# cityflow-project/CityFlow

Measured on AMD Instinct MI355X. Metric: vehicle_steps_per_sec, higher is better.
Workload: dtype f64; 1 GPU; grid_30x30 (reference generator, --tlPlan, interval 1.0) + 3000 seeded interior flows (1 veh / 6 s each until t=240 s); single engine; running_vehicles_start=96748, running_vehicles_end=71131, lanes=11160, lane_count_hash_end=cf8592fdc74305bd, backend=hip-gfx950, layout=ring, parallelism=1 gpu

## Files before the change

cityflow_amd/csrc/hip/cfx_kernels.h:

```cpp
#pragma once

#include "cfx_device.h"

namespace cfxd {

constexpr int kBlock = 256;
#ifndef CFX_ACT_BLOCK
#define CFX_ACT_BLOCK 64
#endif
#ifndef CFX_CROSS_BLOCK
#define CFX_CROSS_BLOCK 256
#endif
constexpr int kActBlock = CFX_ACT_BLOCK;
constexpr int kCrossBlock = CFX_CROSS_BLOCK;
#ifndef CFX_LDS_TEMPL
#define CFX_LDS_TEMPL 32
#endif
constexpr int kLdsTempl = CFX_LDS_TEMPL;
template <class T> __device__ __forceinline__ T ldsRead(const T *p) { return *(const __attribute__((address_space(3))) T *) p; }
template <bool GT>
__device__ __forceinline__ const cfx_vehicle_template *templatesOf(const DevTables &t, cfx_vehicle_template *sT) {
    if constexpr (GT) {
        return t.templ;
    } else {
        const int nd = t.nTempl * (int) (sizeof(cfx_vehicle_template) / sizeof(double));
        const double *src = (const double *) t.templ;
        double *dst = (double *) sT;
        for (int i = threadIdx.x; i < nd; i += blockDim.x) dst[i] = src[i];
        return sT;
    }
}
#ifndef CFX_SCATTER_WAVES
#define CFX_SCATTER_WAVES 0
#endif
#ifndef CFX_SCAN_WAVES
#define CFX_SCAN_WAVES 0
#endif
#if CFX_SCAN_WAVES > 0
#define CFX_SCAN_BOUNDS __launch_bounds__(kBlock, CFX_SCAN_WAVES)
#else
#define CFX_SCAN_BOUNDS __launch_bounds__(kBlock)
#endif
#if CFX_SCATTER_WAVES > 0
#define CFX_SCATTER_BOUNDS __launch_bounds__(kBlock, CFX_SCATTER_WAVES)
#else
#define CFX_SCATTER_BOUNDS
#endif

struct VidTable {
    int32_t *priority, *templ, *route, *nextWait;
    double *enterTime;
    double *customSpeed;
    double *gapState;
    uint8_t *state;
    uint8_t *pendingCustom;
    int32_t *firstNext;
};
constexpr int kFirstNextUnknown = -3;
template <class C>
__device__ __forceinline__ void admittedNext(const C &c, int fn, int lane, int road, int laneIdx, int route, int *next, int *onLast) {
    if (fn != kFirstNextUnknown) {
        *next = fn >= 0 ? fn : -1;
        *onLast = fn == -2 ? 2 : 0;
        return;
    }
    const int base = c.t.routeStart[route];
    if (c.t.routeRoads[base] == road) {
        const int ll = c.t.nextLL[c.t.nextStart[base] + laneIdx];
        *next = ll < 0 ? -1 : c.n.L + ll;
    } else {
        *next = nextOf(c.n, c.t, lane, route, 0);
    }
    *onLast = (*next < 0 && isLastRoad(c, lane, route)) ? 2 : 0;
}

struct DevScalars {
    long long active;
    long long finishedCnt;
    double cumulativeTravelTime;
    long long vehicleSteps;
    int nFinishedStep;
    int overflow;
    int nCrossJobs;
    int nLeftUncounted;
    int ringNearFull;
    int actionMaxT;
    long long tieEvents;
    int tieDrv[8];
    long long admitPending[2];
    int crossJobsStep;
    int crossMultiPass;
    int crossMaxPasses;
    int actionMultiPass;
};

struct HostMirror {
    DevScalars sc;
    int32_t slots;
    int32_t pad;
    unsigned long long progress;
};

struct CompactScratch {
    int32_t *leaveCnt;
    int32_t *maxLeaveIdx;
    int32_t *inCnt;
    int32_t *inHead;
    int32_t *inNext;
};

constexpr int kJobShards = 16;
constexpr int kJobShardStride = 32;
constexpr int kFinShards = 16;
struct FinMap {
    int end[kFinShards];
};
__device__ inline int finMapLoad(FinMap &m, const int32_t *finCount, int finCap) {
    if (threadIdx.x == 0) {
        const int capShard = finCap / kFinShards;
        int run = 0;
        for (int i = 0; i < kFinShards; ++i) {
            run += min(finCount[i * 32], capShard);
            m.end[i] = run;
        }
    }
    __syncthreads();
    return m.end[kFinShards - 1];
}
__device__ __forceinline__ int finAt(const FinMap &m, int finCap, int i) {
    int sh = 0;
    while (i >= m.end[sh]) ++sh;
    return sh * (finCap / kFinShards) + (i - (sh ? m.end[sh - 1] : 0));
}
__device__ __forceinline__ void finCountsClear(int32_t *finCount) {
    for (int i = 0; i < kFinShards; ++i) finCount[i * 32] = 0;
}
__device__ __forceinline__ int finPlace(int32_t *finCount, int finCap) {
    const int shard = blockIdx.x & (kFinShards - 1), capShard = finCap / kFinShards;
    const int idx = atomicAdd(&finCount[shard * 32], 1);
    return idx < capShard ? shard * capShard + idx : -1;
}

struct JobQueue {
    int32_t *count;
    int32_t *jobs;
    int capacity;
    int32_t *overflow;
};

struct ActionBuf {
    double *dis, *speed;
    int32_t *drv;
    int32_t *blocker;
};

__global__ void k_spawn_link(const cfx_spawn *recs, int n, int firstNewVid, VidTable vt, int32_t *waitHead, LcDev lc) {
    int i = blockIdx.x * blockDim.x + threadIdx.x;
    if (i >= n) return;
    cfx_spawn r = recs[i];
    if (lc.on) lcInitVid(lc, r.vid);
    vt.priority[r.vid] = r.priority;
    vt.templ[r.vid] = r.templ;
    vt.route[r.vid] = r.route;
    vt.enterTime[r.vid] = r.enter_time;
    vt.state[r.vid] = 0;
    vt.pendingCustom[r.vid] = 0;
    vt.firstNext[r.vid] = kFirstNextUnknown;
    if (r.lane < 0) return;
    if (r.prev_wait < 0) {
        waitHead[r.lane] = r.vid;
    } else if (r.prev_wait >= firstNewVid) {
        vt.nextWait[r.prev_wait] = r.vid;
    } else if (vt.state[r.prev_wait] != 0) {
        waitHead[r.lane] = r.vid;
    } else {
        vt.nextWait[r.prev_wait] = r.vid;
    }
}

__device__ __forceinline__ int lcNaiveSegment(const StepCtx &c, int lane, double dis) {
    const int nSeg = c.lc.laneNumSegs[lane];
// ... 3082 lines not shown
```

cityflow_amd/csrc/hip/cfx_ring_kernels.h:

```cpp
#pragma once

#include <type_traits>

#include "cfx_kernels.h"


namespace cfxd {

struct RingCtx {
#ifndef CFX_RING_CROSS2_WAVES
#define CFX_RING_CROSS2_WAVES 5
#endif
    static constexpr int kCross2Waves = CFX_RING_CROSS2_WAVES;
    DevNet n;
    DevTables t;
    SlotArrays s;
    double2 *kin;
    double2 *kinN;
    int4 *meta;
    const int2 *blkR;
    int2 *blkW;
    int32_t *slotOf;
    const uint8_t *vState;
    const int2 *ringGeo;
// ... 88 lines not shown
}
__device__ __forceinline__ double2 ntLoad2(const double2 *p) {
    const cfx_v2d v = __builtin_nontemporal_load((const cfx_v2d *) p);
    return make_double2(v.x, v.y);
}
__device__ __forceinline__ void ntStore4(int4 *p, int4 x) {
    const cfx_v4i v = {x.x, x.y, x.z, x.w};
    __builtin_nontemporal_store(v, (cfx_v4i *) p);
}
__device__ __forceinline__ void ntStore2(double2 *p, double a, double b) {
    const cfx_v2d v = {a, b};
    __builtin_nontemporal_store(v, (cfx_v2d *) p);
}

struct RingOut {
    double2 *kinN;
    int2 *blk;
    int4 *scratch;
    MoverRec *movers;
    DevScalars *sc;
    long long *finKey;
    int32_t *finVid;
    int finCap;
    int32_t *finCount;
    __device__ __forceinline__ void park(int s, double v, double iv) const { kinN[s] = make_double2(iv, v); }
    __device__ __forceinline__ double parkedSpeed(int s) const { return kinN[s].y; }
    __device__ __forceinline__ double parkedInterSpeed(int s) const { return kinN[s].x; }
    __device__ __forceinline__ void keep(int s, double dis, double speed) const { kinN[s] = make_double2(dis, speed); }
};
constexpr int kRingIdxBits = 20;

template <bool LC>
__device__ inline void finishAction(const RingCtx &c, const RingOut &o, const cfx_vehicle_template &t, int s, int d, int ,
                                    double speed, double dis, double dlen, int nd0, double v, int blockerSlot, int idx = -1,
                                    int nNow = -1, LeaverPrefetch lp = LeaverPrefetch{false, 0.0, 0, 0, 0}, int flags = -1) {
    static_assert(!LC, "the ring layout does not run lane change");
    v = min2(v, 100);
    if (nd0 < 0) {
        const bool lastRoad = flags >= 0 ? (flags & 2) != 0 : isLastRoad(c, d, c.s.route[s]);
        if (!lastRoad) v = min2(v, noCollisionSpeed(0, 1, speed, t.max_neg_acc, dlen - dis, c.interval, t.min_gap));
    }
    v = max2(v, speed - t.max_neg_acc * c.interval);
    double deltaDis;
    if (v < 0) {
        deltaDis = 0.5 * speed * speed / t.max_neg_acc;
        v = 0;
    } else {
        deltaDis = (speed + v) * c.interval / 2;
    }
    double ndis = deltaDis + dis;
    int newDrv = -1;
    if (ndis > dlen) {
        if (!lp.valid) {
            lp.nextLen = nd0 >= 0 ? c.n.drvLength[nd0] : 0.0;
            lp.vid = c.s.vid[s];
            lp.route = c.s.route[s];
            lp.routePos = c.s.routePos[s];
        }
        ndis -= dlen;
        int drivable = nd0;
        newDrv = drivable >= 0 ? drivable : -2;
        if (drivable >= 0 && ndis > lp.nextLen) {
            int nxt = nextOf(c.n, c.t, drivable, lp.route, lp.routePos);
            for (;;) {
                ndis -= c.n.drvLength[drivable];
                drivable = nxt;
                newDrv = drivable >= 0 ? drivable : -2;
                if (drivable < 0 || !(ndis > c.n.drvLength[drivable])) break;
                nxt = nextOf(c.n, c.t, drivable, lp.route, lp.routePos);
            }
        }
    }
    const int bv = blockerSlot >= 0 ? (lp.blockerVidP2 > 0 ? lp.blockerVidP2 - 2 : c.s.vid[blockerSlot]) : -1;
    if (idx < 0) {
        const int2 geo = c.ringGeo[d];
        idx = (s - geo.x - c.head[d]) & geo.y;
        nNow = cntNow(c, d);
    }
    if (newDrv == -1) {
        if (CFX_KL_NT & 4) ntStore2(&o.kinN[s], ndis, v);
        else o.kinN[s] = make_double2(ndis, v);
        if (bv >= 0) o.blk[s] = make_int2(bv, c.step);
        if (idx == nNow - 1) {
            TailRec r;
            r.dis = ndis;
            r.speed = v;
            r.slot = s;
            r.templ = lp.templP1 > 0 ? lp.templP1 - 1 : c.meta[s].x;
            r.prevDrv = lp.prevValid ? lp.prevDrv : c.s.prevDrv[s];
            r.tag = c.step;
            c.tailW[d] = r;
        }
        return;
    }
    o.kinN[s].y = -1.0;
    atomicAdd(&o.scratch[d].x, 1);
    atomicMax(&o.scratch[d].y, idx);
    if (newDrv >= 0) {
        MoverRec r;
        r.vid = lp.vid;
        r.templ = lp.templP1 > 0 ? lp.templP1 - 1 : c.meta[s].x;
        r.route = lp.route;
        r.routePos = lp.routePos;
        r.oldDrv = d;
        r.newDrv = newDrv;
        r.blockerVid = bv;
        r.dis = ndis;
        r.speed = v;
        atomicAdd(&o.scratch[newDrv].w, 1);
        r.nextIn = atomicExch(&o.scratch[newDrv].z, s);
        o.movers[s] = r;
    } else {
        const int f = finPlace(o.finCount, o.finCap);
        if (f >= 0) {
            o.finKey[f] = ((long long) d << kRingIdxBits) | idx;
            o.finVid[f] = lp.vid;
        } else {
            o.sc->overflow = 1;
        }
    }
}

static_assert(sizeof(SpawnBatch) + sizeof(RingCtx) + sizeof(VidTable) + 256 <= 8192, "kr_admit's arguments: a few KB (the runtime takes 32 KB and more, tools/kernarg_probe.hip)");

struct RingCommit {
    int4 *scratch;
    const MoverRec *movers;
    int32_t *waitHead;
    int32_t *curPhase;
    double *remain;
    int rlTrafficLight, nMaskWords;
    DevScalars *sc;
    const long long *finKey;
    const int32_t *finVid;
    double *finTerm;
    int finCap;
    int32_t *jobCount;
    HostMirror *hostMirror;
    int32_t *finTicket;
    int nStatBlocks;
    uint8_t *vStateW;
    int32_t *slotOfW;
    int exactTimes;
    int lightsDone;
    int32_t *hostCnt;
    int32_t *finCount;
};
struct CommitOut {
    int touched, head, n, tailWritten;
    int entrants;
    TailRec tail;
};
__device__ inline void commitDrivable(const RingCtx &c, const RingCommit &k, const int d, CommitOut *out = nullptr);
__device__ inline void commitStatBlock(const RingCtx &c, const RingCommit &k, const VidTable &vt, int part);
__device__ inline int commitStatBlocks(const RingCommit &k);
__device__ inline void commitClearMasks(const RingCtx &c, const RingCommit &k, int gid, int stride);

struct RingHalo {
    int on;
    const int32_t *cutIndex;
    HaloDev h;
    HaloIO io;
    long long *activeOut;
};

__device__ inline int ringHaloGlobalPrev(const RingCtx &c, const HaloDev &h, int prevDrv) {
    if (prevDrv >= c.n.L) return h.llGlobal[prevDrv - c.n.L];
    if (prevDrv <= -2) return -prevDrv - 2;
    return -1;
}

__device__ inline void ringHaloExport(const RingCtx &c, const RingCommit &k, const RingHalo &rh, int d, int ci, const CommitOut &co) {
    const HaloDev &h = rh.h;
    const int2 geo = c.ringGeo[d];
    int head = co.touched ? co.head : c.head[d];
    int n = co.touched ? co.n : c.cnt[d];
    if (ci < h.nGhost) {
        char *blk = rh.io.send[h.ghostPeer[ci]] + h.ghostSendOff[ci];
        const int in = co.entrants;
        int m = in;
        if (m > CFX_HALO_MAX_MIGRANTS) {
            m = CFX_HALO_MAX_MIGRANTS;
            k.sc->overflow = 3;
        }
        ((int32_t *) blk)[0] = m;
        ((int32_t *) blk)[1] = 0;
        HaloMigrant *rec = (HaloMigrant *) (blk + 8);
        for (int j = 0; j < m; ++j) {
            const int s = ringSlot(geo, head, n - in + j);
            const double2 kv = c.kinN[s];
            HaloMigrant r;
            r.vid = c.s.vid[s];
            r.routePos = c.s.routePos[s];
            r.prevLL = ringHaloGlobalPrev(c, h, c.s.prevDrv[s]);
            r.pad = 0;
            r.dis = kv.x;
            r.speed = kv.y;
            rec[j] = r;
        }
        h.ghostHadEntrants[ci] = in > 0;
        if (in > 0) {
            for (int j = 0; j + 1 < n; ++j) c.slotOf[c.s.vid[ringSlot(geo, head, j)]] = -1;
            head = (head + n - 1) & geo.y;
            c.head[d] = head;
            c.cnt[d] = 1;
            atomicAdd((unsigned long long *) rh.activeOut, (unsigned long long) in);
        }
        return;
    }
    const int j = ci - h.nGhost;
    if (j < h.nImport) {
        HaloTail t;
        t.vid = -1;
        t.prevLL = -1;
        t.dis = 0.0;
        t.speed = 0.0;
        if (n > 0) {
            const int s = ringSlot(geo, head, n - 1);
            const double2 kv = c.kinN[s];
            t.vid = c.s.vid[s];
            t.prevLL = ringHaloGlobalPrev(c, h, c.s.prevDrv[s]);
            t.dis = kv.x;
            t.speed = kv.y;
        }
        *(HaloTail *) (rh.io.send[h.importPeer[j]] + h.importSendOff[j]) = t;
    }
}

__device__ inline void ringHaloWriteTail(const RingCtx &c, int lane, int slot) {
    TailRec r{};
    r.slot = -1;
    if (slot >= 0) {
        const double2 kv = c.kin[slot];
        r.dis = kv.x;
        r.speed = kv.y;
        r.slot = slot;
        r.templ = c.meta[slot].x;
        r.prevDrv = c.s.prevDrv[slot];
    }
    r.tag = c.step - 1;
    const_cast<TailRec *>(c.tailR)[lane] = r;
}

__device__ inline void ringHaloImportCut(const RingCtx &c, const HaloDev &h, const HaloIO &io, const VidTable &vt, DevScalars *sc, int i) {
    if (i < h.nImport) {
        const int l = h.importLane[i];
        const char *blk = io.recv[h.importPeer[i]] + h.importRecvOff[i];
        const int m = ((const int32_t *) blk)[0];
        if (m <= 0) return;
        const HaloMigrant *rec = (const HaloMigrant *) (blk + 8);
        const int2 geo = c.ringGeo[l];
        const int head = c.head[l], n = c.cnt[l];
        if (n + m > geo.y) {
            sc->overflow = 8;
            return;
        }
        const int road = c.n.laneRoad[l];
        int last = -1;
        for (int j = 0; j < m; ++j) {
            const HaloMigrant r = rec[j];
            const int s = ringSlot(geo, head, n + j);
            const int route = vt.route[r.vid];
            const int next = nextOf(c.n, c.t, l, route, r.routePos);
            const int base = c.t.routeStart[route], len = c.t.routeStart[route + 1] - base;
            const int onLast = (next < 0 && c.t.routeRoads[base + len - 1] == road) ? 2 : 0;
            c.s.vid[s] = r.vid;
            c.s.drv[s] = l;
            c.s.prevDrv[s] = r.prevLL >= 0 ? -(r.prevLL + 2) : -1;
            c.s.routePos[s] = r.routePos;
            c.s.route[s] = route;
            c.meta[s] = make_int4(vt.templ[r.vid], next, onLast, CFX_INT_MAX);
            c.kin[s] = make_double2(r.dis, r.speed);
            const_cast<int2 *>(c.blkR)[s] = make_int2(-1, -1);
            c.slotOf[r.vid] = s;
            vt.state[r.vid] = 1;
            last = s;
        }
        c.cnt[l] = n + m;
        atomicAdd((unsigned long long *) &sc->active, (unsigned long long) m);
        ringHaloWriteTail(c, l, last);
        return;
    }
    const int j = i - h.nImport;
    if (j < h.nGhost && !h.ghostHadEntrants[j]) {
        const int g = h.ghostLane[j];
        const HaloTail t = *(const HaloTail *) (io.recv[h.ghostPeer[j]] + h.ghostRecvOff[j]);
        const int2 geo = c.ringGeo[g];
        const int head = c.head[g], n = c.cnt[g];
        for (int q = 0; q < n; ++q) {
            const int v = c.s.vid[ringSlot(geo, head, q)];
            if (v != t.vid) c.slotOf[v] = -1;
        }
        if (t.vid < 0) {
            c.cnt[g] = 0;
            ringHaloWriteTail(c, g, -1);
            return;
        }
        int prev = -1;
        if (t.prevLL >= 0) {
            const int k = h.llLocalOfGlobal[t.prevLL];
            prev = k >= 0 ? c.n.L + k : -(t.prevLL + 2);
        }
        const int s = ringSlot(geo, head, 0);
        c.s.vid[s] = t.vid;
        c.s.drv[s] = g;
        c.s.prevDrv[s] = prev;
        c.s.routePos[s] = 0;
        c.s.route[s] = vt.route[t.vid];
        c.meta[s] = make_int4(vt.templ[t.vid], -1, 0, CFX_INT_MAX);
        c.kin[s] = make_double2(t.dis, t.speed);
        const_cast<int2 *>(c.blkR)[s] = make_int2(-1, -1);
        c.slotOf[t.vid] = s;
        c.cnt[g] = 1;
        ringHaloWriteTail(c, g, s);
    }
}

__device__ inline bool ringHaloWaitPeer(const HaloIO &io, int p, DevScalars *sc) {
    unsigned spins = 0;
    while (__hip_atomic_load(io.waitFlag[p], __ATOMIC_ACQUIRE, __HIP_MEMORY_SCOPE_SYSTEM) < io.epoch) {
        if (++spins > (1u << 22)) {
            sc->overflow = 4;
            return false;
        }
        __builtin_amdgcn_s_sleep(16);
    }
    return true;
}

struct RingHaloIn {
    int on;
    const int32_t *cutIndex;
    HaloDev h;
    HaloIO io;
    long long *activeOut;
};

__global__ void kr_halo_import(RingCtx c, HaloDev h, HaloIO io, VidTable vt, DevScalars *sc, long long *activeOut) {
    if (io.nWait > 0) {
        __shared__ int ok;
        if (threadIdx.x == 0) {
            ok = 1;
            for (int p = 0; p < io.nWait && ok; ++p) ok = ringHaloWaitPeer(io, p, sc) ? 1 : 0;
        }
        __syncthreads();
        if (!ok) return;
    }
    const int i = blockIdx.x * blockDim.x + threadIdx.x;
    if (i == 0) {
        const long long out = *activeOut;
        if (out) {
            *activeOut = 0;
            atomicAdd((unsigned long long *) &sc->active, (unsigned long long) (-out));
        }
    }
    if (i < h.nImport + h.nGhost) ringHaloImportCut(c, h, io, vt, sc, i);
}

template <bool COMMIT, int NB = kAdmitRecs, class Batch = SpawnBatchT<NB>, bool GT = false>
__global__ __launch_bounds__(kBlock) void kr_admit(RingCtx cIn, int32_t *admitStep, int32_t *waitHead, VidTable vt, DevScalars *sc,
                                                   const Batch batch, const RingCommit k, const RingHaloIn hin) {
    constexpr bool kMem = std::is_same<Batch, SpawnBatchMem>::value;
    const int d = blockIdx.x * blockDim.x + threadIdx.x;
    const bool isLane = d < cIn.n.L, inRange = d < cIn.n.L + cIn.n.K;
    int b0 = 0, b1 = 0;
    if constexpr (kMem) {
        if ((int) blockIdx.x < batch.nLaneBlocks) {
            b0 = batch.blockOff[blockIdx.x];
            b1 = batch.blockOff[blockIdx.x + 1];
        }
    }
    TailRec committed{};
    int w = -1, n = 0, head = 0, road = 0, laneIdx = 0;
    int2 geo = make_int2(0, 0);
    int wt = 0, route = 0, nextWait = -1, fn = kFirstNextUnknown;
    uint8_t pending = 0;
    if constexpr (COMMIT) {
        const int nBody = (int) gridDim.x - commitStatBlocks(k);
        if ((int) blockIdx.x >= nBody) {
            commitStatBlock(cIn, k, vt, (int) blockIdx.x - nBody);
            return;
        }
        commitClearMasks(cIn, k, d, nBody * (int) blockDim.x);
        if (inRange) committed = cIn.tailW[d];
        if (isLane) {
            w = waitHead[d];
            if (admitStep[d] == cIn.step) w = cIn.admitRec[d].y;
            n = cIn.cnt[d];
            geo = cIn.ringGeo[d];
            head = cIn.head[d];
            road = cIn.n.laneRoad[d];
            laneIdx = cIn.n.laneIndex[d];
            if (w >= 0) {
                wt = vt.templ[w];
                route = vt.route[w];
                nextWait = vt.nextWait[w];
                pending = vt.pendingCustom[w];
                fn = vt.firstNext[w];
            }
        }
        if (inRange) {
            CommitOut co;
            commitDrivable(cIn, k, d, &co);
            if (co.touched) {
                head = co.head;
                n = co.n;
                if (co.tailWritten) committed = co.tail;
            }
        }
    }
    RingCtx c = cIn;
    if constexpr (!COMMIT) {
        if (hin.on) {
            if (d == 0) {
                const long long out = *hin.activeOut;
                if (out) {
                    *hin.activeOut = 0;
                    atomicAdd((unsigned long long *) &sc->active, (unsigned long long) (-out));
                }
            }
            const int ci = isLane ? hin.cutIndex[d] : -1;
            if (ci >= 0) {
                const int nG = hin.h.nGhost;
                const int peer = ci < nG ? hin.h.ghostPeer[ci] : hin.h.importPeer[ci - nG];
                if (hin.io.nWait == 0 || ringHaloWaitPeer(hin.io, peer, sc))
                    ringHaloImportCut(c, hin.h, hin.io, vt, sc, ci < nG ? hin.h.nImport + ci : ci - nG);
            }
        }
    }
    if constexpr (COMMIT) {
        c.step = cIn.step + 1;
        c.tailR = cIn.tailW;
        c.tailW = const_cast<TailRec *>(cIn.tailR);
        c.kin = cIn.kinN;
        c.kinN = cIn.kin;
        c.blkR = cIn.blkW;
        c.blkW = const_cast<int2 *>(cIn.blkR);
    }
    __shared__ int sAdmitted;
    __shared__ cfx_vehicle_template sT[kLdsTempl];
    __shared__ int sLane[NB];
    const int nRecs = batch.n, firstNewVid = batch.firstNewVid;
    if (threadIdx.x == 0) sAdmitted = 0;
    if constexpr (kMem) {
        for (int i = threadIdx.x; i < b1 - b0 && i < NB; i += blockDim.x) sLane[i] = batch.lane[b0 + i];
    } else {
        for (int i = threadIdx.x; i < nRecs; i += blockDim.x) sLane[i] = batch.lane[i];
    }
    auto laneOfRec = [&](int j) {
        if constexpr (kMem) return j - b0 < NB ? ldsRead(&sLane[j - b0]) : batch.lane[j];
        else return sLane[j];
    };
    const int recLo = kMem ? b0 : 0, recHi = kMem ? b1 : nRecs;
    const cfx_vehicle_template *const tv = templatesOf<GT>(c.t, sT);
    if constexpr (!COMMIT) {
        if (inRange) committed = c.tailR[d];
        if (isLane) {
            w = waitHead[d];
            n = c.cnt[d];
            geo = c.ringGeo[d];
            head = c.head[d];
            road = c.n.laneRoad[d];
            laneIdx = c.n.laneIndex[d];
        }
        if (w >= 0) {
            wt = vt.templ[w];
            route = vt.route[w];
            nextWait = vt.nextWait[w];
            pending = vt.pendingCustom[w];
            fn = vt.firstNext[w];
        }
    }
    __syncthreads();
    if (nRecs > 0) {
        auto writeRows = [&](int from, int to) {
            for (int i = from + (int) threadIdx.x; i < to; i += blockDim.x) {
                const int v = firstNewVid + batch.vidOff[i];
                vt.priority[v] = batch.priority[i];
                vt.templ[v] = batch.templ[i];
                vt.route[v] = batch.route[i];
                vt.enterTime[v] = batch.enterTime;
                vt.state[v] = 0;
                vt.pendingCustom[v] = 0;
                vt.firstNext[v] = batch.firstNext[i];
            }
        };
        if constexpr (kMem) {
            writeRows(blockIdx.x == 0 ? 0 : b0, b1);
        } else {
            if (blockIdx.x == 0) writeRows(0, nRecs);
        }
        if (isLane) {
            int lo = recLo, hi = recHi;
            while (lo < hi) {
                const int mid = (lo + hi) >> 1;
                if (laneOfRec(mid) < d) lo = mid + 1;
                else hi = mid;
            }
            int headRec = -1;
            for (int j = lo; j < recHi && laneOfRec(j) == d; ++j) {
                const int pv = batch.prevWait[j], v = firstNewVid + batch.vidOff[j];
                bool becomesHead = pv < 0;
                if (pv >= firstNewVid) vt.nextWait[pv] = v;
                else if (pv >= 0) {
                    if (vt.state[pv] != 0) becomesHead = true;
                    else vt.nextWait[pv] = v;
                }
                if (becomesHead) headRec = j;
            }
            if (headRec >= 0) {
                w = firstNewVid + batch.vidOff[headRec];
                wt = batch.templ[headRec];
                route = batch.route[headRec];
                fn = batch.firstNext[headRec];
                pending = 0;
                nextWait = -1;
                waitHead[d] = w;
            }
            if (w >= 0)
                for (int j = lo; j < recHi && laneOfRec(j) == d; ++j)
                    if (batch.prevWait[j] == w) nextWait = firstNewVid + batch.vidOff[j];
        }
    }
    if (inRange) {
        TailRec now = committed;
        if (committed.tag != c.step - 1) now.slot = -1;
        if (!isLane) {
            const int k = d - c.n.L, in = c.n.llInter[k];
            const int ph = c.curPhase[in];
            if (c.gatePhase[((c.step + 1) & 1) * c.n.I + in] != ph) {
                const int flags = (c.n.phaseAvail[c.n.interAvailStart[in] + ph * c.n.interNRL[in] + c.n.llRoadLink[k]] != 0 ? 1 : 0) |
                                  (c.n.llType[k] << 1) | (c.n.llXStart[k + 1] > c.n.llXStart[k] ? 8 : 0);
                c.llGate[k] = make_int4(flags, c.n.llEndLane[k], c.n.llXStart[k], c.n.llXStart[k + 1]);
            }
            if (c.n.llLocal[k] == 0) c.gatePhase[(c.step & 1) * c.n.I + in] = ph;
        } else {
            const int lane = d;
            bool admit = w >= 0;
            if (admit && now.slot >= 0 && !(now.dis > tv[now.templ].len + tv[wt].min_gap)) admit = false;
            if (admit && n >= geo.y) {
                sc->overflow = 8;
                admit = false;
            }
            if (admit) {
                int next, onLast;
                admittedNext(c, fn, lane, road, laneIdx, route, &next, &onLast);
                const int slot = ringSlot(geo, head, n);
                const double v0 = tv[wt].initial_speed;
                c.s.vid[slot] = w;
                c.s.drv[slot] = lane;
                c.s.prevDrv[slot] = -1;
                c.s.routePos[slot] = 0;
                c.s.route[slot] = route;
                c.meta[slot] = make_int4(wt, next, pending | onLast, CFX_INT_MAX);
                c.kin[slot] = make_double2(0.0, v0);
                c.slotOf[w] = slot;
                c.admitRec[lane] = make_int2(w, nextWait);
                admitStep[lane] = c.step;
                now.dis = 0.0;
                now.speed = v0;
                now.slot = slot;
                now.templ = wt;
                now.prevDrv = -1;
                if (!(c.n.laneGhost && c.n.laneGhost[lane])) atomicAdd(&sAdmitted, 1);
            }
        }
        now.tag = c.step;
        c.tailNow[d] = now;
    }
    __syncthreads();
    if (threadIdx.x == 0 && sAdmitted) atomicAdd((unsigned long long *) &sc->admitPending[c.step & 1], (unsigned long long) sAdmitted);
}

__device__ inline void llstateRing(const RingCtx &c, int k) {
    if (k >= c.n.K) return;
    const int d = c.n.L + k;
    const int endLane = c.n.llEndLane[k], startLane = c.n.llStartLane[k];
    const Tail tu = tailNowOf(c, endLane);
    const int u = (tu.slot >= 0 && tu.prevDrv == d) ? tu.slot : -1;
    int f = cntNow(c, startLane) > 0 ? firstSlot(c, startLane) : -1;
    const bool green = (c.llGate[k].x & 1) != 0;
    if (f >= 0 && !(green && c.meta[f].y == d)) f = -1;
    const int nOn = c.cnt[d];
    c.llDyn[k] = make_int4(u, f, firstSlot(c, d), nOn);
    if (u >= 0 || f >= 0 || nOn > 0) {
        LLAux a{};
        a.uDis = tu.dis;
        a.uSpeed = tu.speed;
        a.uTempl = tu.templ;
        if (f >= 0) {
            const double2 kf = c.kin[f];
            a.fDis = kf.x;
            a.fSpeed = kf.y;
            a.fTempl = c.meta[f].x;
        }
        a.llLen = c.n.drvLength[d];
        a.startLen = c.n.drvLength[startLane];
        c.llAux[k] = a;
        const int in = c.n.llInter[k];
        const int bit = c.n.llLocal[k];
        atomicOr(&c.interMask[c.n.interMaskStart[in] + (bit >> 6)], 1ULL << (bit & 63));
    }
}

__device__ __forceinline__ int blockerOfNotified(const RingCtx &c, const Notified &nf) {
    if (!nf.pre) return blockerOf(c, nf.slot);
    return (nf.blk.x >= 0 && nf.blk.y == c.step - 1) ? c.slotOf[nf.blk.x] : -1;
}
__device__ __forceinline__ void notifiedExtras(const RingCtx &c, Notified &nf) {
    nf.enterLLT = c.meta[nf.slot].w;
    nf.blk = c.blkR[nf.slot];
    nf.vid = c.s.vid[nf.slot];
    nf.pre = true;
}
__device__ inline Notified notifiedFrom(const RingCtx &c, const cfx_vehicle_template *tv, int k, double x, const int4 dyn,
                                        const LLAux &a);
__device__ inline Notified notified(const RingCtx &c, const cfx_vehicle_template *tv, int k, double x) {
    const int4 dyn = c.llDyn[k];
    const LLAux a = c.llAux[k];
    return notifiedFrom(c, tv, k, x, dyn, a);
}
__device__ inline Notified notifiedFrom(const RingCtx &c, const cfx_vehicle_template *tv, int k, double x, const int4 dyn,
                                        const LLAux &a) {
    Notified nf{-1, 0, 0.0, 0.0, false, 0, make_int2(-1, -1)};
    if (dyn.x < 0 && dyn.y < 0 && dyn.w == 0) return nf;
    if (dyn.x >= 0) {
        const double vehDistance = a.uDis - tv[a.uTempl].len;
        const double crossDistance = a.llLen - x;
        if (crossDistance + vehDistance < 0.0) {
            nf.slot = dyn.x;
            nf.templ = a.uTempl;
            nf.speed = a.uSpeed;
            nf.dist = -(a.uDis + crossDistance);
            notifiedExtras(c, nf);
            return nf;
        }
    }
    if (dyn.w > 0) {
        const SegWalk walk = segWalk(c, c.n.L + k, dyn.z);
        for (int i = 0; i < dyn.w; i += 2) {
            const int w0 = walk.at(i), w1 = walk.at(i + 1 < dyn.w ? i + 1 : i);
            const double2 k0 = c.kin[w0], k1 = c.kin[w1];
            const int t0 = c.meta[w0].x, t1 = c.meta[w1].x;
            for (int q = 0; q < 2 && i + q < dyn.w; ++q) {
                const int w = q ? w1 : w0;
                const double2 kw = q ? k1 : k0;
                const double vehDistance = kw.x;
                const int wt = q ? t1 : t0;
                if (!(vehDistance > x) || (vehDistance - x - tv[wt].len <= 0.0)) {
                    nf.slot = w;
                    nf.templ = wt;
                    nf.speed = kw.y;
                    nf.dist = x - vehDistance;
                    notifiedExtras(c, nf);
                    return nf;
                }
            }
        }
    }
    if (dyn.y >= 0) {
        nf.slot = dyn.y;
        nf.templ = a.fTempl;
        nf.speed = a.fSpeed;
        nf.dist = (a.startLen - a.fDis) + x;
        notifiedExtras(c, nf);
    }
    return nf;
}

__device__ inline Notified notifiedEagerFrom(const RingCtx &c, const cfx_vehicle_template *tv, int k, double x, const int4 dyn,
                                        const LLAux &a) {
    Notified nf{-1, 0, 0.0, 0.0, false, 0, make_int2(-1, -1)};
    if (dyn.x < 0 && dyn.y < 0 && dyn.w == 0) return nf;
    const SegWalk walk = segWalk(c, c.n.L + k, dyn.z);
    const bool haveU = dyn.x >= 0, haveOn = dyn.w > 0;
    const int w0 = haveOn ? walk.at(0) : 0, w1 = haveOn ? walk.at(dyn.w > 1 ? 1 : 0) : 0;
    double2 k0 = make_double2(0.0, 0.0), k1 = k0;
    int4 m0 = make_int4(0, 0, 0, 0), m1 = m0;
    int2 b0 = make_int2(-1, -1);
    int v0 = 0;
    if (haveOn) {
        k0 = c.kin[w0];
        k1 = c.kin[w1];
        m0 = c.meta[w0];
        m1 = c.meta[w1];
        b0 = c.blkR[w0];
        v0 = c.s.vid[w0];
    }
    bool found = false, extras = false;
    if (haveU) {
        const double vehDistance = a.uDis - tv[a.uTempl].len;
        const double crossDistance = a.llLen - x;
        if (crossDistance + vehDistance < 0.0) {
            nf.slot = dyn.x;
            nf.templ = a.uTempl;
            nf.speed = a.uSpeed;
            nf.dist = -(a.uDis + crossDistance);
            found = extras = true;
        }
    }
    if (!found && haveOn) {
        for (int q = 0; q < 2 && q < dyn.w && !found; ++q) {
            const double2 kw = q ? k1 : k0;
            const int4 mw = q ? m1 : m0;
            const double vehDistance = kw.x;
            if (!(vehDistance > x) || (vehDistance - x - tv[mw.x].len <= 0.0)) {
                nf.slot = q ? w1 : w0;
                nf.templ = mw.x;
                nf.speed = kw.y;
                nf.dist = x - vehDistance;
                found = true;
                if (q == 0) {
                    nf.enterLLT = mw.w;
                    nf.blk = b0;
                    nf.vid = v0;
                    nf.pre = true;
                } else {
                    extras = true;
                }
            }
        }
        for (int i = 2; i < dyn.w && !found; i += 2) {
            const int x0 = walk.at(i), x1 = walk.at(i + 1 < dyn.w ? i + 1 : i);
            const double2 q0 = c.kin[x0], q1 = c.kin[x1];
// ... 676 lines not shown
    if ((t & 63) == 0 && qv > 0) ls = list[qv - 1].x;
    if (w * kListBlock >= total) return;
    const cfx_vehicle_template *const tv = templatesOf<GT>(c.t, sT);
    if (!GT) __syncthreads();
    const bool valid = qv < total;
    const int lane = t & 63;
    const int slot = valid ? e.x : 0, d = e.y, idx = valid ? e.z : 0;
    KSTAMP(11, 1);
    SlotIn in;
    in.vid = 0;
    in.dis = 0.0;
    in.speed = 0.0;
    in.templIdx = 0;
    in.nd0 = -1;
    in.flags = 0;
    double2 kp = make_double2(0.0, 0.0);
    int tp = 0;
    double2 lm = make_double2(0.0, 0.0);
    int4 hop = make_int4(-2, -2, -2, -2), en = make_int4(-1, -1, -1, -1);
    if (valid) {
        const double2 kv = (CFX_KL_NT & 8) ? ntLoad2(&c.kin[slot]) : c.kin[slot];
        const int4 mv = (CFX_KL_NT & 16) ? ntLoad4(&c.meta[slot]) : c.meta[slot];
        lm = c.n.drvLM[d];
        if (d < c.n.L) {
            hop = c.n.laneLL4[d];
            en = c.n.laneEnd4[d];
        }
        if (idx > 0 && lane == 0) {
            kp = c.kin[ls];
            tp = c.meta[ls].x;
        }
        in.dis = kv.x;
        in.speed = kv.y;
        in.templIdx = mv.x;
        in.nd0 = mv.y;
        in.flags = mv.z;
        in.lastRoadFlags = mv.z;
    }
    const int slotUp = __shfl_up(slot, 1, 64);
    const double disUp = __shfl_up(in.dis, 1, 64), speedUp = __shfl_up(in.speed, 1, 64);
    const int templUp = __shfl_up(in.templIdx, 1, 64);
    if (!valid) return;
    if (lane != 0) ls = slotUp;
    in.d = d;
    in.head = idx == 0;
    in.idx = idx;
    in.nNow = e.w & 0x7fffffff;
    in.leaderSlot = idx > 0 ? ls : 0;
    in.disPrev = lane == 0 ? kp.x : disUp;
    in.speedPrev = lane == 0 ? kp.y : speedUp;
    in.templPrev = lane == 0 ? tp : templUp;
    if (in.flags & (kFlagCustom | kFlagStateGap)) {
        in.vid = c.s.vid[slot];
        c.meta[slot].z = in.flags & ~(kFlagCustom | kFlagStateGap);
    }
    in.lm = lm;
    in.hop = make_int4(-2, -2, -2, -2);
    in.endLane = -1;
    if (in.nd0 >= c.n.L) {
        in.hop = hop;
        const int ll = in.nd0 - c.n.L;
        in.endLane = hop.x == ll ? en.x : (hop.y == ll ? en.y : (hop.z == ll ? en.z : (hop.w == ll ? en.w : -1)));
    }
    in.laneAdmitted = e.w < 0;
    const RingPush push{q, jobRecs, c.n.L};
    KSTAMP(11, 2);
    actionOneRounds<GHOST>(c, o, tv, slot, in, push);
    KSTAMP(11, 3);
}


__device__ inline void ringCopySlot(const RingCtx &c, int from, int to) {
    c.s.vid[to] = c.s.vid[from];
    c.s.drv[to] = c.s.drv[from];
    c.s.prevDrv[to] = c.s.prevDrv[from];
    c.s.routePos[to] = c.s.routePos[from];
    c.s.route[to] = c.s.route[from];
    c.meta[to] = c.meta[from];
    c.blkW[to] = c.blkW[from];
    c.kinN[to] = c.kinN[from];
    c.slotOf[c.s.vid[from]] = to;
}

__device__ inline bool ringFinishStatistics(const RingCtx &c, const VidTable &vt, const RingCommit &k, int part, int nParts) {
    __shared__ long long fin[kFinLds];
    __shared__ double term[kFinLds];
    __shared__ int lastShared;
    __shared__ FinMap fm;
    DevScalars *sc = k.sc;
    const int F = finMapLoad(fm, k.finCount, k.finCap);
    const double now = c.step * c.interval;
    auto foldAdmissions = [&]() {
        const long long a = sc->admitPending[c.step & 1];
        sc->admitPending[c.step & 1] = 0;
        sc->vehicleSteps += a;
        sc->active += a;
    };
    if (k.exactTimes) {
        const bool lastBlock = exactFinishStatistics(now, vt, sc, F, [&](int i) { return k.finVid[finAt(fm, k.finCap, i)]; }, k.vStateW,
                                                     k.finTicket, part, nParts, 0, k.finCount, k.slotOfW);
        if (lastBlock && threadIdx.x == 0) foldAdmissions();
        return lastBlock;
    }
    const bool inLds = nParts == 1 && F <= kFinLds;
    const int per = (F + nParts - 1) / nParts;
    const int lo = part * per, hi = min(F, lo + per);
    for (int base = lo; base < hi; base += blockDim.x) {
        const int i = base + (int) threadIdx.x;
        const int at = i < hi ? finAt(fm, k.finCap, i) : 0;
        const long long me = i < hi ? k.finKey[at] : 0;
        int rank = 0;
        for (int cb = 0; cb < F; cb += kFinLds) {
            const int cn = min(kFinLds, F - cb);
            __syncthreads();
            for (int j = threadIdx.x; j < cn; j += blockDim.x) fin[j] = k.finKey[finAt(fm, k.finCap, cb + j)];
            __syncthreads();
            if (i < hi)
                for (int j = 0; j < cn; ++j) rank += fin[j] < me;
        }
        if (i < hi) {
            const int vid = k.finVid[at];
            const double tt = now - vt.enterTime[vid];
            k.vStateW[vid] = 2;
            k.slotOfW[vid] = -1;
            if (inLds) term[rank] = tt;
            else k.finTerm[rank] = tt;
        }
    }
    bool last = true;
    if (nParts > 1) {
        __threadfence();
        __syncthreads();
        if (threadIdx.x == 0) lastShared = atomicAdd(k.finTicket, 1) == nParts - 1;
        __syncthreads();
        last = lastShared != 0;
        if (!last) return false;
        if (threadIdx.x == 0) *k.finTicket = 0;
        __threadfence();
    }
    __syncthreads();
    const double cum = orderedSum(sc->cumulativeTravelTime, F, term, k.finTerm, inLds);
    if (threadIdx.x == 0) {
        sc->cumulativeTravelTime = cum;
        sc->vehicleSteps += sc->active;
        sc->finishedCnt += F;
        sc->active -= F;
        finCountsClear(k.finCount);
        foldAdmissions();
    }
    return last;
}

__device__ inline void commitDrivable(const RingCtx &c, const RingCommit &k, const int d, CommitOut *out) {
    const int4 sc = k.scratch[d];
    const bool admitted = d < c.n.L && c.admitStep[d] == c.step;
    if (out) {
        out->touched = 0;
        out->entrants = 0;
    }
    if (!admitted && sc.x == 0 && sc.z < 0) return;
    const int2 geo = c.ringGeo[d];
    int head = c.head[d];
    int n = c.cnt[d];
    if (admitted) {
        const int2 rec = c.admitRec[d];
        k.waitHead[d] = rec.y;
        k.vStateW[rec.x] = 1;
        n += 1;
    }
    if (sc.x > 0) {
        if (sc.y + 1 != sc.x) {
            int wr = n - 1;
            for (int r = n - 1; r >= 0; --r) {
                const int from = ringSlot(geo, head, r);
                if (c.kinN[from].y < 0.0) continue;
                if (wr != r) ringCopySlot(c, from, ringSlot(geo, head, wr));
                --wr;
            }
        }
        head = (head + sc.x) & geo.y;
        n -= sc.x;
    }
    int m = 0, tailRank = -1;
    TailRec tail{};
    for (int e = sc.z; e >= 0; e = k.movers[e].nextIn) {
        const MoverRec r = k.movers[e];
        int rank = 0;
        for (int f = sc.z; f >= 0; f = k.movers[f].nextIn) {
            if (f == e) continue;
            const double od = k.movers[f].dis;
            const bool tieBefore = od == r.dis && k.movers[f].vid < r.vid;
            rank += (od > r.dis) || tieBefore;
            if (tieBefore) k.sc->tieDrv[atomicAdd((unsigned long long *) &k.sc->tieEvents, 1ULL) & 7ULL] = d;
        }
        ++m;
        if (n + rank > geo.y) {
            k.sc->overflow = 8;
            continue;
        }
        const int slot = ringSlot(geo, head, n + rank);
        int rp = r.routePos;
        c.s.vid[slot] = r.vid;
        c.s.drv[slot] = d;
        c.s.prevDrv[slot] = r.oldDrv;
        c.s.route[slot] = r.route;
        c.blkW[slot] = make_int2(r.blockerVid, c.step);
        int next, enterLLT, onLast = 0;
        if (d < c.n.L) {
            enterLLT = CFX_INT_MAX;
            const int base = c.t.routeStart[r.route], len = c.t.routeStart[r.route + 1] - base;
            const int road = c.n.laneRoad[d], laneIdx = c.n.laneIndex[d];
            const int p0 = rp < len ? rp : len - 1, p1 = rp + 1 < len ? rp + 1 : len - 1;
            const int road0 = c.t.routeRoads[base + p0], road1 = c.t.routeRoads[base + p1];
            int row = c.t.nextStart[base + p0];
            const int row1 = c.t.nextStart[base + p1], roadLast = c.t.routeRoads[base + len - 1];
            if (rp < len && road0 != road) {
                ++rp;
                row = row1;
                if (rp < len && road1 != road) {
                    ++rp;
                    while (rp < len && c.t.routeRoads[base + rp] != road) ++rp;
                    if (rp < len) row = c.t.nextStart[base + rp];
                }
            }
            next = -1;
            if (rp < len) {
                const int ll = c.t.nextLL[row + laneIdx];
                next = ll < 0 ? -1 : c.n.L + ll;
            }
            if (next < 0 && road == roadLast) onLast = 2;
        } else {
            enterLLT = c.step;
            next = c.n.llEndLane[d - c.n.L];
        }
        c.s.routePos[slot] = rp;
        c.meta[slot] = make_int4(r.templ, next, onLast, enterLLT);
        c.kinN[slot] = make_double2(r.dis, r.speed);
        c.slotOf[r.vid] = slot;
        if (rank > tailRank) {
            tailRank = rank;
            tail.dis = r.dis;
            tail.speed = r.speed;
            tail.slot = slot;
            tail.templ = r.templ;
            tail.prevDrv = r.oldDrv;
        }
    }
    n += m;
    if (tailRank >= 0) {
        tail.tag = c.step;
        c.tailW[d] = tail;
    } else if (sc.x > 0) {
        if (n == 0) {
            tail.slot = -1;
        } else {
            const int ts = ringSlot(geo, head, n - 1);
            const double2 kt = c.kinN[ts];
            tail.dis = kt.x;
            tail.speed = kt.y;
            tail.slot = ts;
            tail.templ = c.meta[ts].x;
            tail.prevDrv = c.s.prevDrv[ts];
        }
        tail.tag = c.step;
        c.tailW[d] = tail;
    }
    if (n > geo.y) k.sc->overflow = 8;
    else if (n + min(8, (geo.y + 1) / 2) > geo.y) k.sc->ringNearFull = 1;
    c.head[d] = head;
    c.cnt[d] = n;
    if (k.hostCnt && d < c.n.L) k.hostCnt[d] = n;
    k.scratch[d] = make_int4(0, -1, -1, 0);
    if (out) {
        out->touched = 1;
        out->head = head;
        out->n = n;
        out->tailWritten = (tailRank >= 0 || sc.x > 0) ? 1 : 0;
        out->entrants = m;
        out->tail = tail;
    }
}

__device__ inline int commitStatBlocks(const RingCommit &k) { return k.nStatBlocks; }
__device__ inline void commitStatBlock(const RingCtx &c, const RingCommit &k, const VidTable &vt, int part) {
    if (part == 0 && threadIdx.x < kJobShards) k.jobCount[threadIdx.x * kJobShardStride] = 0;
    const bool last = ringFinishStatistics(c, vt, k, part, k.nStatBlocks);
    if (last && threadIdx.x == 0 && k.hostMirror) {
        k.hostMirror->sc = *k.sc;
        k.sc->actionMaxT = 0;
        k.hostMirror->slots = (int32_t) k.sc->active;
        __hip_atomic_store(&k.hostMirror->progress, ((unsigned long long) (c.step + 1) << 32) | (unsigned) k.sc->active,
                           __ATOMIC_RELAXED, __HIP_MEMORY_SCOPE_SYSTEM);
    }
}
__device__ inline void commitClearMasks(const RingCtx &c, const RingCommit &k, int gid, int stride) {
    for (int i = gid; i < k.nMaskWords; i += stride) c.interMask[i] = 0ULL;
}

__global__ __launch_bounds__(kBlock) void kr_commit(RingCtx c, RingCommit k, VidTable vt, RingHalo rh) {
    const int nBody = (int) gridDim.x - k.nStatBlocks;
    if ((int) blockIdx.x >= nBody) {
        commitStatBlock(c, k, vt, (int) blockIdx.x - nBody);
        return;
    }
    const int gid = blockIdx.x * blockDim.x + threadIdx.x;
    const int stride = nBody * blockDim.x;
    commitClearMasks(c, k, gid, stride);
    if (!k.rlTrafficLight && !k.lightsDone) passTimeAll(c.n, k.curPhase, k.remain, c.interval, gid, stride);
    const int D = c.n.L + c.n.K;
    for (int d = gid; d < D; d += stride) {
        CommitOut co;
        commitDrivable(c, k, d, &co);
        if (rh.on && d < c.n.L) {
            const int ci = rh.cutIndex[d];
            if (ci >= 0) {
                ringHaloExport(c, k, rh, d, ci, co);
                if (rh.io.nSignal > 0) {
                    const int nCut = rh.h.nGhost + rh.h.nImport;
                    __threadfence_system();
                    if (atomicAdd(rh.io.ticket, 1) == nCut - 1) {
                        __threadfence_system();
                        *rh.io.ticket = 0;
                        for (int p = 0; p < rh.io.nSignal; ++p)
                            __hip_atomic_store(rh.io.signalFlag[p], rh.io.epoch, __ATOMIC_RELEASE, __HIP_MEMORY_SCOPE_SYSTEM);
                    }
                }
            }
        }
    }
}

struct RingDense {
    int32_t *vid, *drv, *prevDrv, *blockerVid, *enterLLT, *routePos, *leaderVid;
    uint8_t *flags;
    double *dis, *speed, *gap;
};

__global__ void kr_gather(RingCtx c, const int32_t *off, RingDense out, int wantLeader) {
    const int d = blockIdx.x * blockDim.x + threadIdx.x;
    if (d >= c.n.L + c.n.K) return;
    const int n = c.cnt[d];
    if (n == 0) return;
    const int2 geo = c.ringGeo[d];
    const int head = c.head[d], o = off[d];
    for (int i = 0; i < n; ++i) {
        const int s = ringSlot(geo, head, i);
        out.vid[o + i] = c.s.vid[s];
        out.drv[o + i] = d;
        out.prevDrv[o + i] = c.s.prevDrv[s];
        out.blockerVid[o + i] = blockerVid(c, s);
        const double2 kv = c.kin[s];
        const int4 mv = c.meta[s];
        out.enterLLT[o + i] = mv.w;
        out.routePos[o + i] = c.s.routePos[s];
        out.flags[o + i] = (uint8_t) (mv.z & (kFlagCustom | kFlagStateGap));
        out.dis[o + i] = kv.x;
        out.speed[o + i] = kv.y;
        if (wantLeader) {
            double gap = 0;
            int ls;
            if (i > 0) {
                ls = ringSlot(geo, head, i - 1);
                gap = c.kin[ls].x - c.t.templ[c.meta[ls].x].len - kv.x;
            } else {
                ls = findHeadLeader(c, c.t.templ, s, d, kv.x, c.t.templ[mv.x].approach_dist, mv.y, c.n.drvLength[d], &gap).slot;
            }
            if ((mv.z & kFlagStateGap) && ls >= 0) gap = c.vGapState[c.s.vid[s]];
            out.leaderVid[o + i] = ls >= 0 ? c.s.vid[ls] : -1;
            out.gap[o + i] = gap;
        }
    }
}

__global__ void kr_scatter_in(RingCtx c, const int32_t *off, RingDense in, VidTable vt) {
    const int d = blockIdx.x * blockDim.x + threadIdx.x;
    if (d >= c.n.L + c.n.K) return;
    const int n = off[d + 1] - off[d];
    c.head[d] = 0;
    c.cnt[d] = n;
    const int2 geo = c.ringGeo[d];
    for (int i = 0; i < n; ++i) {
        const int s = geo.x + i, j = off[d] + i;
        const int v = in.vid[j];
        const int route = vt.route[v];
        c.s.vid[s] = v;
        c.s.drv[s] = d;
// ... 392 lines not shown
```

Baseline: 2.121 billion vehicle-steps/s.

## Hoist commit-phase global loads in kr_admit ahead of the block barrier

Restructures the COMMIT path of kr_admit so that the per-lane loads (scratch, ring geometry, head, count, admit record, first mover record, link-lane tables, phase values) are all issued up front, alongside the template and lane-batch staging. The commit itself then runs from those preloaded values via a new commitDrivableWith, and the barrier is moved so the loads can be in flight together. It also adds an explicit vmcnt(0) wait on early-returning stat blocks, moves the mask clearing to the end of the kernel, and caches each mover's next link in the ranking loops. The aim is to overlap global-memory latency that was previously serialised. In exchange it raises register pressure and adds a gfx9-only compile guard plus a pile of bitmask compile switches.

Measured after the change: 2.191 billion vehicle-steps/s (median of 6 runs). 1.03x the previous value.

```diff
diff --git a/cityflow_amd/csrc/hip/cfx_kernels.h b/cityflow_amd/csrc/hip/cfx_kernels.h
--- a/cityflow_amd/csrc/hip/cfx_kernels.h
+++ b/cityflow_amd/csrc/hip/cfx_kernels.h
@@ -18,15 +18,33 @@
 #endif
 constexpr int kLdsTempl = CFX_LDS_TEMPL;
 template <class T> __device__ __forceinline__ T ldsRead(const T *p) { return *(const __attribute__((address_space(3))) T *) p; }
+__device__ __forceinline__ int templDoubles(const DevTables &t) { return t.nTempl * (int) (sizeof(cfx_vehicle_template) / sizeof(double)); }
 template <bool GT>
 __device__ __forceinline__ const cfx_vehicle_template *templatesOf(const DevTables &t, cfx_vehicle_template *sT) {
     if constexpr (GT) {
         return t.templ;
     } else {
-        const int nd = t.nTempl * (int) (sizeof(cfx_vehicle_template) / sizeof(double));
+        const int nd = templDoubles(t);
         const double *src = (const double *) t.templ;
         double *dst = (double *) sT;
         for (int i = threadIdx.x; i < nd; i += blockDim.x) dst[i] = src[i];
+        return sT;
+    }
+}
+template <bool GT> __device__ __forceinline__ double templatesRequest(const DevTables &t) {
+    if constexpr (GT) return 0.0;
+    else return (int) threadIdx.x < templDoubles(t) ? ((const double *) t.templ)[threadIdx.x] : 0.0;
+}
+template <bool GT>
+__device__ __forceinline__ const cfx_vehicle_template *templatesStage(const DevTables &t, cfx_vehicle_template *sT, double first) {
+    if constexpr (GT) {
+        return t.templ;
+    } else {
+        const int nd = templDoubles(t);
+        const double *src = (const double *) t.templ;
+        double *dst = (double *) sT;
+        if ((int) threadIdx.x < nd) dst[threadIdx.x] = first;
+        for (int i = threadIdx.x + blockDim.x; i < nd; i += blockDim.x) dst[i] = src[i];
         return sT;
     }
 }
diff --git a/cityflow_amd/csrc/hip/cfx_ring_kernels.h b/cityflow_amd/csrc/hip/cfx_ring_kernels.h
--- a/cityflow_amd/csrc/hip/cfx_ring_kernels.h
+++ b/cityflow_amd/csrc/hip/cfx_ring_kernels.h
@@ -264,6 +264,16 @@
     TailRec tail;
 };
 __device__ inline void commitDrivable(const RingCtx &c, const RingCommit &k, const int d, CommitOut *out = nullptr);
+struct CommitPre {
+    int4 sc;
+    int admitted;
+    int2 rec;
+    int2 geo;
+    int head, n;
+    int llNext;
+    MoverRec first;
+};
+__device__ inline void commitDrivableWith(const RingCtx &c, const RingCommit &k, const int d, const CommitPre &pre, CommitOut *out);
 __device__ inline void commitStatBlock(const RingCtx &c, const RingCommit &k, const VidTable &vt, int part);
 __device__ inline int commitStatBlocks(const RingCommit &k);
 __device__ inline void commitClearMasks(const RingCtx &c, const RingCommit &k, int gid, int stride);
@@ -469,12 +479,29 @@
     if (i < h.nImport + h.nGhost) ringHaloImportCut(c, h, io, vt, sc, i);
 }
 
+#if defined(__HIP_DEVICE_COMPILE__) && !defined(__GFX9__)
+#error "kWaitVmcnt0 is the gfx9 encoding of s_waitcnt"
+#endif
+#ifndef CFX_ADMIT_PIECES
+#define CFX_ADMIT_PIECES 47
+#endif
+constexpr int kAdmitPieces = CFX_ADMIT_PIECES;
+constexpr int kWaitVmcnt0 = (0x0 << 0) | (0x0 << 14) | (0x7 << 4) | (0xF << 8);
+static_assert(kWaitVmcnt0 == 0x0F70, "s_waitcnt vmcnt(0) expcnt(7) lgkmcnt(15)");
+#if defined(CFX_TRACE) && CFX_TRACE_KERNEL == 12
+#define ASTAMP(k) if (threadIdx.x == 0) g_trace[(size_t) (8192 + blockIdx.x) * 8 + (k)] = (long long) wall_clock64()
+#define ANOTE(k, v) if (threadIdx.x == 0) g_trace[(size_t) (8192 + blockIdx.x) * 8 + (k)] = (long long) (v)
+#else
+#define ASTAMP(k)
+#define ANOTE(k, v)
+#endif
 template <bool COMMIT, int NB = kAdmitRecs, class Batch = SpawnBatchT<NB>, bool GT = false>
 __global__ __launch_bounds__(kBlock) void kr_admit(RingCtx cIn, int32_t *admitStep, int32_t *waitHead, VidTable vt, DevScalars *sc,
                                                    const Batch batch, const RingCommit k, const RingHaloIn hin) {
     constexpr bool kMem = std::is_same<Batch, SpawnBatchMem>::value;
     const int d = blockIdx.x * blockDim.x + threadIdx.x;
     const bool isLane = d < cIn.n.L, inRange = d < cIn.n.L + cIn.n.K;
+    ASTAMP(0);
     int b0 = 0, b1 = 0;
     if constexpr (kMem) {
         if ((int) blockIdx.x < batch.nLaneBlocks) {
@@ -487,39 +514,19 @@
     int2 geo = make_int2(0, 0);
     int wt = 0, route = 0, nextWait = -1, fn = kFirstNextUnknown;
     uint8_t pending = 0;
+    int llIn = 0, llEnd = -1, llFirst = 0;
+    CommitPre pre{};
+    pre.sc = make_int4(0, -1, -1, 0);
     if constexpr (COMMIT) {
         const int nBody = (int) gridDim.x - commitStatBlocks(k);
         if ((int) blockIdx.x >= nBody) {
             commitStatBlock(cIn, k, vt, (int) blockIdx.x - nBody);
+            ANOTE(5, 2);
+            ASTAMP(3);
+            if constexpr ((kAdmitPieces & 8) != 0) __builtin_amdgcn_s_waitcnt(kWaitVmcnt0);
             return;
         }
-        commitClearMasks(cIn, k, d, nBody * (int) blockDim.x);
-        if (inRange) committed = cIn.tailW[d];
-        if (isLane) {
-            w = waitHead[d];
-            if (admitStep[d] == cIn.step) w = cIn.admitRec[d].y;
-            n = cIn.cnt[d];
-            geo = cIn.ringGeo[d];
-            head = cIn.head[d];
-            road = cIn.n.laneRoad[d];
-            laneIdx = cIn.n.laneIndex[d];
-            if (w >= 0) {
-                wt = vt.templ[w];
-                route = vt.route[w];
-                nextWait = vt.nextWait[w];
-                pending = vt.pendingCustom[w];
-                fn = vt.firstNext[w];
-            }
-        }
-        if (inRange) {
-            CommitOut co;
-            commitDrivable(cIn, k, d, &co);
-            if (co.touched) {
-                head = co.head;
-                n = co.n;
-                if (co.tailWritten) committed = co.tail;
-            }
-        }
+        if constexpr ((kAdmitPieces & 32) == 0) commitClearMasks(cIn, k, d, nBody * (int) blockDim.x);
     }
     RingCtx c = cIn;
     if constexpr (!COMMIT) {
@@ -553,37 +560,83 @@
     __shared__ cfx_vehicle_template sT[kLdsTempl];
     __shared__ int sLane[NB];
     const int nRecs = batch.n, firstNewVid = batch.firstNewVid;
+    const int stBase = kMem ? b0 : 0, stN = kMem ? min(b1 - b0, NB) : nRecs;
+    const double tFirst = templatesRequest<GT>(c.t);
+    int lFirst = 0;
+    if ((int) threadIdx.x < stN) lFirst = batch.lane[stBase + threadIdx.x];
+    if (inRange) committed = c.tailR[d];
+    if (inRange && !isLane) {
+        const int kk = d - c.n.L;
+        llIn = c.n.llInter[kk];
+        llEnd = c.n.llEndLane[kk];
+        llFirst = c.n.llLocal[kk] == 0;
+    }
+    if constexpr (COMMIT) {
+        if (inRange) {
+            pre.sc = k.scratch[d];
+            pre.n = c.cnt[d];
+            pre.geo = c.ringGeo[d];
+            pre.head = c.head[d];
+            pre.llNext = llEnd;
+        }
+    }
+    if (isLane) {
+        w = waitHead[d];
+        if constexpr (COMMIT) {
+            pre.admitted = admitStep[d] == cIn.step;
+            pre.rec = c.admitRec[d];
+            n = pre.n;
+            geo = pre.geo;
+            head = pre.head;
+        } else {
+            n = c.cnt[d];
+            geo = c.ringGeo[d];
+            head = c.head[d];
+        }
+        road = c.n.laneRoad[d];
+        laneIdx = c.n.laneIndex[d];
+    }
     if (threadIdx.x == 0) sAdmitted = 0;
-    if constexpr (kMem) {
-        for (int i = threadIdx.x; i < b1 - b0 && i < NB; i += blockDim.x) sLane[i] = batch.lane[b0 + i];
-    } else {
-        for (int i = threadIdx.x; i < nRecs; i += blockDim.x) sLane[i] = batch.lane[i];
-    }
+    if ((int) threadIdx.x < stN) sLane[threadIdx.x] = lFirst;
+    for (int i = threadIdx.x + blockDim.x; i < stN; i += blockDim.x) sLane[i] = batch.lane[stBase + i];
     auto laneOfRec = [&](int j) {
         if constexpr (kMem) return j - b0 < NB ? ldsRead(&sLane[j - b0]) : batch.lane[j];
         else return sLane[j];
     };
     const int recLo = kMem ? b0 : 0, recHi = kMem ? b1 : nRecs;
-    const cfx_vehicle_template *const tv = templatesOf<GT>(c.t, sT);
-    if constexpr (!COMMIT) {
-        if (inRange) committed = c.tailR[d];
-        if (isLane) {
-            w = waitHead[d];
-            n = c.cnt[d];
-            geo = c.ringGeo[d];
-            head = c.head[d];
-            road = c.n.laneRoad[d];
-            laneIdx = c.n.laneIndex[d];
-        }
-        if (w >= 0) {
-            wt = vt.templ[w];
-            route = vt.route[w];
-            nextWait = vt.nextWait[w];
-            pending = vt.pendingCustom[w];
-            fn = vt.firstNext[w];
-        }
-    }
-    __syncthreads();
+    const cfx_vehicle_template *const tv = templatesStage<GT>(c.t, sT, tFirst);
+    if constexpr (COMMIT) {
+        if (pre.admitted) w = pre.rec.y;
+        if constexpr ((kAdmitPieces & 2) != 0)
+            if (pre.sc.z >= 0) pre.first = k.movers[pre.sc.z];
+    }
+    if (w >= 0) {
+        wt = vt.templ[w];
+        route = vt.route[w];
+        nextWait = vt.nextWait[w];
+        pending = vt.pendingCustom[w];
+        fn = vt.firstNext[w];
+    }
+    int ph = 0, gatePh = 0;
+    if (inRange && !isLane) {
+        ph = c.curPhase[llIn];
+        gatePh = c.gatePhase[((c.step + 1) & 1) * c.n.I + llIn];
+    }
+    if constexpr (!COMMIT || (kAdmitPieces & 1) != 0) __syncthreads();
+    ASTAMP(1);
+    if constexpr (COMMIT) {
+        if (inRange) {
+            CommitOut co;
+            commitDrivableWith(cIn, k, d, pre, &co);
+            if (co.touched) {
+                head = co.head;
+                n = co.n;
+                if (co.tailWritten) committed = co.tail;
+            }
+        }
+        if constexpr ((kAdmitPieces & 1) == 0) __syncthreads();
+    }
+    ASTAMP(2);
     if (nRecs > 0) {
         auto writeRows = [&](int from, int to) {
             for (int i = from + (int) threadIdx.x; i < to; i += blockDim.x) {
@@ -638,14 +691,13 @@
         TailRec now = committed;
         if (committed.tag != c.step - 1) now.slot = -1;
         if (!isLane) {
-            const int k = d - c.n.L, in = c.n.llInter[k];
-            const int ph = c.curPhase[in];
-            if (c.gatePhase[((c.step + 1) & 1) * c.n.I + in] != ph) {
+            const int k = d - c.n.L, in = llIn;
+            if (gatePh != ph) {
                 const int flags = (c.n.phaseAvail[c.n.interAvailStart[in] + ph * c.n.interNRL[in] + c.n.llRoadLink[k]] != 0 ? 1 : 0) |
                                   (c.n.llType[k] << 1) | (c.n.llXStart[k + 1] > c.n.llXStart[k] ? 8 : 0);
-                c.llGate[k] = make_int4(flags, c.n.llEndLane[k], c.n.llXStart[k], c.n.llXStart[k + 1]);
-            }
-            if (c.n.llLocal[k] == 0) c.gatePhase[(c.step & 1) * c.n.I + in] = ph;
+                c.llGate[k] = make_int4(flags, llEnd, c.n.llXStart[k], c.n.llXStart[k + 1]);
+            }
+            if (llFirst) c.gatePhase[(c.step & 1) * c.n.I + in] = ph;
         } else {
             const int lane = d;
             bool admit = w >= 0;
@@ -680,8 +732,11 @@
         now.tag = c.step;
         c.tailNow[d] = now;
     }
+    if constexpr (COMMIT && (kAdmitPieces & 32) != 0) commitClearMasks(cIn, k, d, ((int) gridDim.x - commitStatBlocks(k)) * (int) blockDim.x);
     __syncthreads();
     if (threadIdx.x == 0 && sAdmitted) atomicAdd((unsigned long long *) &sc->admitPending[c.step & 1], (unsigned long long) sAdmitted);
+    ANOTE(5, ((int) (blockIdx.x + 1) * (int) blockDim.x > c.n.L) ? 1 : 0);
+    ASTAMP(3);
 }
 
 __device__ inline void llstateRing(const RingCtx &c, int k) {
@@ -1664,18 +1719,39 @@
 }
 
 __device__ inline void commitDrivable(const RingCtx &c, const RingCommit &k, const int d, CommitOut *out) {
-    const int4 sc = k.scratch[d];
-    const bool admitted = d < c.n.L && c.admitStep[d] == c.step;
+    CommitPre pre{};
+    pre.sc = k.scratch[d];
+    pre.admitted = d < c.n.L && c.admitStep[d] == c.step;
+    if (!pre.admitted && pre.sc.x == 0 && pre.sc.z < 0) {
+        if (out) {
+            out->touched = 0;
+            out->entrants = 0;
+        }
+        return;
+    }
+    pre.geo = c.ringGeo[d];
+    pre.head = c.head[d];
+    pre.n = c.cnt[d];
+    pre.llNext = d >= c.n.L ? c.n.llEndLane[d - c.n.L] : -1;
+    if (pre.admitted) pre.rec = c.admitRec[d];
+    if constexpr ((kAdmitPieces & 2) != 0)
+        if (pre.sc.z >= 0) pre.first = k.movers[pre.sc.z];
+    commitDrivableWith(c, k, d, pre, out);
+}
+__device__ inline void commitDrivableWith(const RingCtx &c, const RingCommit &k, const int d, const CommitPre &pre, CommitOut *out) {
+    const int4 sc = pre.sc;
+    const bool admitted = pre.admitted != 0;
+    const int llNext = pre.llNext;
     if (out) {
         out->touched = 0;
         out->entrants = 0;
     }
     if (!admitted && sc.x == 0 && sc.z < 0) return;
-    const int2 geo = c.ringGeo[d];
-    int head = c.head[d];
-    int n = c.cnt[d];
+    const int2 geo = pre.geo;
+    int head = pre.head;
+    int n = pre.n;
     if (admitted) {
-        const int2 rec = c.admitRec[d];
+        const int2 rec = pre.rec;
         k.waitHead[d] = rec.y;
         k.vStateW[rec.x] = 1;
         n += 1;
@@ -1695,13 +1771,20 @@
     }
     int m = 0, tailRank = -1;
     TailRec tail{};
-    for (int e = sc.z; e >= 0; e = k.movers[e].nextIn) {
-        const MoverRec r = k.movers[e];
+    for (int e = sc.z, eNext; e >= 0; e = (kAdmitPieces & 4) != 0 ? eNext : k.movers[e].nextIn) {
+        MoverRec r = pre.first;
+        if ((kAdmitPieces & 2) == 0 || e != sc.z) r = k.movers[e];
+        eNext = r.nextIn;
         int rank = 0;
-        for (int f = sc.z; f >= 0; f = k.movers[f].nextIn) {
-            if (f == e) continue;
+        for (int f = sc.z, fNext; f >= 0; f = fNext) {
+            if (f == e) {
+                fNext = (kAdmitPieces & 4) != 0 ? r.nextIn : k.movers[f].nextIn;
+                continue;
+            }
             const double od = k.movers[f].dis;
-            const bool tieBefore = od == r.dis && k.movers[f].vid < r.vid;
+            const int ov = k.movers[f].vid;
+            fNext = k.movers[f].nextIn;
+            const bool tieBefore = od == r.dis && ov < r.vid;
             rank += (od > r.dis) || tieBefore;
             if (tieBefore) k.sc->tieDrv[atomicAdd((unsigned long long *) &k.sc->tieEvents, 1ULL) & 7ULL] = d;
         }
@@ -1743,7 +1826,7 @@
             if (next < 0 && road == roadLast) onLast = 2;
         } else {
             enterLLT = c.step;
-            next = c.n.llEndLane[d - c.n.L];
+            next = llNext;
         }
         c.s.routePos[slot] = rp;
         c.meta[slot] = make_int4(r.templ, next, onLast, enterLLT);
```
